# lauraset/Super-resolution-building-height-estimation

Hardware: AMD Instinct MI355X
Metric: tiles/sec (64x64x8ch->256x256 height) (higher is better)
Workload: dtype f16 operands / f32 accumulate (MFMA), f32 residual stream; 1 GPU; RRDBNet x4 (23 RRDB, 64 feat) forward_feature, batch 32 tiles/GPU, 64x64x3 -> 64x256x256 (BASELINE.json configs[1]); global_batch=32, parallelism=tile-sharded x1 (no data-path collective)

## Files before the change

super-resolution-building-height-estimation_amd/csrc/srbh_ptrunk.hip:

```cpp
#include <stdlib.h>
#include <string.h>
#include <mutex>
#include "srbh_conv3x3_kernel.h"


namespace {
using namespace srbh;
using namespace srbh_k;

struct PLayer {
    const char* w;
    const float* bias;
};

struct PParams {
    char* dense[2];
    long img_b;
    int plane_b, row_b;
    float* xr;
    float* xrr;
    const PLayer* layers;
    int nlayers;
    int H, W, tiles_per_img, nblocks;
    int* prog;
// ... 11 lines not shown
constexpr unsigned SPIN_LIMIT = 4u << 20;
using G = TileGeo<0>;
constexpr int IN_EX = G::UNITS * 16;
constexpr int A_STAGE_B = IN_EX + 18 * 1024, B_STAGE_B = IN_EX + 36 * 1024;
constexpr int A_BASE = IN_EX;
constexpr int A_BIAS_OFF = A_BASE + 2 * A_STAGE_B, B_BIAS_OFF = 2 * B_STAGE_B;
constexpr int P_WORD_OFF = A_BIAS_OFF + 128;
constexpr int P_LDS_B = 163840;
static_assert(P_WORD_OFF + 4 <= P_LDS_B && B_BIAS_OFF + 256 <= P_WORD_OFF, "LDS map must fit 160 KiB");
__device__ __forceinline__ int stage_off(int cb, int idx) { return cb == 1 ? A_BASE + idx * A_STAGE_B : idx * B_STAGE_B; }

#include "srbh_ptrunk3_kernel.h"

}

namespace srbh {

unsigned long long* g_ptrunk_prof = nullptr;
static int g_trunk_timing = 0;
static hipEvent_t g_trunk_ev[2];
static int g_trunk_ev_recorded = 0;
static const char* g_trunk_kernel = "none";

constexpr int MAX_BLOCKS = 64;
static size_t table_bytes() { return ((size_t)MAX_BLOCKS * 15 * sizeof(PLayer) + 255) & ~(size_t)255; }
static size_t prog_bytes(int B, int tpi) { return ((size_t)B * 2 * tpi * sizeof(int) + 255) & ~(size_t)255; }

size_t ptrunk_aux_bytes(int B, int tiles_per_img) { return table_bytes() + 2 * prog_bytes(B, tiles_per_img) + 256; }
__global__ void ptrunk_reset_kernel(int* __restrict__ prog, int* __restrict__ xcc, int* __restrict__ err, int n) {
    const int i = blockIdx.x * blockDim.x + threadIdx.x;
    if (i < n) { prog[i] = 0; xcc[i] = 0; }
    if (i == 0) *err = 0;
}

size_t ptrunk_err_offset(int B, int tiles_per_img) { return table_bytes() + prog_bytes(B, tiles_per_img); }

struct TabEntry {
    int dev;
    std::vector<char> host;
    PLayer* dptr;
};
static std::mutex g_tab_mu;
static std::vector<TabEntry> g_tabs;

static int device_table(const std::vector<PLayer>& tab, PLayer** out) {
    int dev = 0;
    SRBH_HIP(hipGetDevice(&dev));
    const size_t nb = tab.size() * sizeof(PLayer);
    std::lock_guard<std::mutex> lock(g_tab_mu);
    for (size_t i = 0; i < g_tabs.size(); ++i)
        if (g_tabs[i].dev == dev && g_tabs[i].host.size() == nb && memcmp(g_tabs[i].host.data(), tab.data(), nb) == 0) {
            *out = g_tabs[i].dptr;
            return SRBH_OK;
        }
    if (g_tabs.size() >= 16) {
        SRBH_HIP(hipFree(g_tabs.front().dptr));
        g_tabs.erase(g_tabs.begin());
    }
    TabEntry e;
    e.dev = dev;
    e.host.assign((const char*)tab.data(), (const char*)tab.data() + nb);
    SRBH_HIP(hipMalloc(&e.dptr, nb));
    SRBH_HIP(hipMemcpy(e.dptr, tab.data(), nb, hipMemcpyHostToDevice));
    *out = e.dptr;
    g_tabs.push_back(std::move(e));
    return SRBH_OK;
}

int ptrunk_takes(int num_block, int H, int W, int* takes, int* ncu_out) {
    *takes = 0;
    if (W != TILE_W || (H % TILE_H) != 0 || num_block <= 0 || num_block > MAX_BLOCKS) return SRBH_OK;
    int dev = 0;
    SRBH_HIP(hipGetDevice(&dev));
    int ncu = 0;
    SRBH_HIP(hipDeviceGetAttribute(&ncu, hipDeviceAttributeMultiprocessorCount, dev));
    if (ncu_out) *ncu_out = ncu;
    if (H / TILE_H > ncu) return SRBH_OK;
    constexpr int LDS_B = P_LDS_B;
    SRBH_ONCE_PER_DEVICE({
        SRBH_HIP(hipFuncSetAttribute((const void*)ptrunk3_kernel<0>, hipFuncAttributeMaxDynamicSharedMemorySize, LDS_B));
        SRBH_HIP(hipFuncSetAttribute((const void*)ptrunk3_kernel<1>, hipFuncAttributeMaxDynamicSharedMemorySize, LDS_B));
        SRBH_HIP(hipFuncSetAttribute((const void*)ptrunk3_kernel<0, 1>, hipFuncAttributeMaxDynamicSharedMemorySize, LDS_B));
        SRBH_HIP(hipFuncSetAttribute((const void*)ptrunk3_kernel<0, 0, 1>, hipFuncAttributeMaxDynamicSharedMemorySize, LDS_B));
    });
    int per_cu = 0;
    SRBH_HIP(hipOccupancyMaxActiveBlocksPerMultiprocessor(&per_cu, ptrunk3_kernel<0>, 256, LDS_B));
    if (per_cu < 1) return SRBH_OK;
    *takes = 1;
    return SRBH_OK;
}

int ptrunk_run(const srbh_rrdbnet_desc* d, void* dense0, void* dense1, float* xr, float* xrr, int B, int H, int W,
               void* aux, hipStream_t stream, int* used, int* final_cur, long train_stride, const void* mask, long mask_stride, bool bf16) {
    *used = 0;
    if (mask && train_stride <= 0) return SRBH_OK;
    SRBH_REQUIRE(!bf16 || (train_stride == 0 && !mask), "ptrunk_run: the bf16 form is the inference forward only");
    int ncu = 0, takes = 0;
    if (int rc = ptrunk_takes(d->num_block, H, W, &takes, &ncu)) return rc;
    if (!takes) return SRBH_OK;
    const int tpi = H / TILE_H;
    constexpr int LDS_B = P_LDS_B;
    const int nl = d->num_block * 15;
    std::vector<PLayer> tab(nl);
    int cur = 0, li = 0;
    for (int blk = 0; blk < d->num_block; ++blk)
        for (int r = 0; r < 3; ++r) {
            const srbh_conv_w* cw = d->rdb + (blk * 3 + r) * 5;
            for (int k = 0; k < 5; ++k) tab[li++] = PLayer{(const char*)cw[k].w, cw[k].bias};
            cur ^= 1;
        }
    *final_cur = cur;
    char* a = (char*)aux;
    PLayer* d_tab = nullptr;
    if (int rc = device_table(tab, &d_tab)) return rc;
    int* d_prog = (int*)(a + table_bytes());
    int* d_err = (int*)(a + ptrunk_err_offset(B, tpi));
    int* d_xcc = (int*)(a + ptrunk_err_offset(B, tpi) + 256);
    hipLaunchKernelGGL(ptrunk_reset_kernel, dim3((B * tpi + 255) / 256), dim3(256), 0, stream, d_prog, d_xcc, d_err, B * tpi);
    SRBH_HIP(hipGetLastError());
    const Act16Geo g = act16_geo(B, 6, H, W);
    int imgs_per_launch = ncu / tpi;
    if (const char* ie = getenv("SRBH_PT_IMAGES")) {
        const int cap = atoi(ie);
        if (cap > 0 && cap < imgs_per_launch) {
            const int nl_ = (B + cap - 1) / cap;
            imgs_per_launch = (B + nl_ - 1) / nl_;
        }
    }
    for (int b0 = 0; b0 < B; b0 += imgs_per_launch) {
        const int nb = (B - b0) < imgs_per_launch ? (B - b0) : imgs_per_launch;
        PParams pp;
        pp.dense_stride = train_stride;
        pp.keep_all = pp.out_pixel = train_stride > 0;
        pp.mask = mask ? (const char*)mask + (long)b0 * g.img_b : nullptr;
        pp.mask_stride = mask_stride;
        pp.dense[0] = (char*)dense0 + (long)b0 * g.img_b;
        pp.dense[1] = (train_stride > 0 ? (char*)dense0 + train_stride : (char*)dense1) + (long)b0 * g.img_b;
        pp.img_b = g.img_b;
        pp.plane_b = g.plane_b;
        pp.row_b = g.row_b;
        pp.xr = xr + (long)b0 * H * W * 64;
        pp.xrr = xrr + (long)b0 * H * W * 64;
        pp.layers = d_tab;
        pp.nlayers = nl;
        pp.H = H;
        pp.W = W;
        pp.tiles_per_img = tpi;
        pp.nblocks = nb * tpi;
        pp.prog = d_prog + b0 * tpi;
        pp.err = d_err;
        pp.xcc = d_xcc + b0 * tpi;
        {
            const char* e = getenv("SRBH_PT_WT");
            pp.force_wt = (e && atoi(e) == 1) ? 1 : 0;
        }
        if (getenv("SRBH_PT_PROF") && !bf16 && !g_ptrunk_prof)
            SRBH_HIP(hipMalloc(&g_ptrunk_prof, (size_t)ncu * MAX_BLOCKS * 15 * 6 * 8));
        pp.prof = bf16 ? nullptr : g_ptrunk_prof;
        if (g_trunk_timing && b0 == 0) SRBH_HIP(hipEventRecord(g_trunk_ev[0], stream));
        g_trunk_kernel = "ptrunk3_kernel";
        if (mask)
            hipLaunchKernelGGL((ptrunk3_kernel<0, 1>), dim3(pp.nblocks), dim3(256), LDS_B, stream, pp);
        else if (bf16)
            hipLaunchKernelGGL((ptrunk3_kernel<0, 0, 1>), dim3(pp.nblocks), dim3(256), LDS_B, stream, pp);
        else if (pp.prof)
            hipLaunchKernelGGL((ptrunk3_kernel<1>), dim3(pp.nblocks), dim3(256), LDS_B, stream, pp);
        else
            hipLaunchKernelGGL((ptrunk3_kernel<0>), dim3(pp.nblocks), dim3(256), LDS_B, stream, pp);
        SRBH_HIP(hipGetLastError());
    }
    if (g_trunk_timing) { SRBH_HIP(hipEventRecord(g_trunk_ev[1], stream)); g_trunk_ev_recorded = 1; }
    if (getenv("SRBH_PT_PROF") && g_ptrunk_prof && !bf16) {
        SRBH_HIP(hipStreamSynchronize(stream));
        const int nblk = (B < imgs_per_launch ? B : imgs_per_launch) * tpi;
        std::vector<unsigned long long> h((size_t)nblk * nl * 6);
        SRBH_HIP(hipMemcpy(h.data(), g_ptrunk_prof, h.size() * 8, hipMemcpyDeviceToHost));
        double cyc = 0;
        for (int b = 0; b < nblk; ++b) cyc += (double)(h[((size_t)b * nl + nl - 1) * 6 + 2] - h[(size_t)b * nl * 6]);
        fprintf(stderr, "[srbh] ptrunk: avg %.0f shader cycles per workgroup (first layer start -> last epilogue)\n", cyc / nblk);
        double loop[5] = {0}, epi[5] = {0}, pub[5] = {0}, wait[5] = {0}, tot5[5] = {0}, dma[5] = {0}, bar[5] = {0};
        for (int b = 0; b < nblk; ++b)
            for (int L = 1; L + 1 < nl; ++L) {
                const unsigned long long* q = &h[((size_t)b * nl + L) * 6];
                const unsigned long long* qn = &h[((size_t)b * nl + L + 1) * 6];
                const int k = L % 5;
                loop[k] += (double)(q[1] - q[0]); epi[k] += (double)(q[2] - q[1]); pub[k] += (double)(q[3] >> 32);
                wait[k] += (double)(q[3] & 0xffffffffu); tot5[k] += (double)(qn[0] - q[0]);
                bar[k] += (double)q[4]; dma[k] += (double)q[5];
            }
        const double cnt = (double)nblk * (nl - 2) / 5.0;
        for (int k = 0; k < 5; ++k)
            fprintf(stderr, "[srbh]   conv%d: loop %.0f (of which: waiting for the own LDS-DMA %.0f, at the step barriers %.0f; prologue %.0f) | "
                    "epilogue %.0f | publish/seam %.0f | start-to-start %.0f\n",
                    k + 1, loop[k] / cnt, dma[k] / cnt, bar[k] / cnt, wait[k] / cnt, epi[k] / cnt, pub[k] / cnt, tot5[k] / cnt);
        double e5[2] = {0, 0}, s5[2] = {0, 0};
        long n5[2] = {0, 0};
        for (int b = 0; b < nblk; ++b)
            for (int L = 4; L + 1 < nl; L += 5) {
                const unsigned long long* q = &h[((size_t)b * nl + L) * 6];
                const int kind = ((L / 5) % 3) == 2;
                e5[kind] += (double)(q[2] - q[1]); s5[kind] += (double)(q[3] >> 32); n5[kind]++;
            }
        fprintf(stderr, "[srbh]   conv5 epilogue: %.0f plain / %.0f RRDB-closing; seam %.0f / %.0f\n", e5[0] / (n5[0] ? n5[0] : 1),
                e5[1] / (n5[1] ? n5[1] : 1), s5[0] / (n5[0] ? n5[0] : 1), s5[1] / (n5[1] ? n5[1] : 1));
    }
    *used = 1;
    return SRBH_OK;
}

}

extern "C" int srbh_trunk_timing(int on) {
    using namespace srbh;
    if (on && !g_trunk_timing) {
        SRBH_HIP(hipEventCreate(&g_trunk_ev[0]));
        SRBH_HIP(hipEventCreate(&g_trunk_ev[1]));
    } else if (!on && g_trunk_timing) {
        SRBH_HIP(hipEventDestroy(g_trunk_ev[0]));
        SRBH_HIP(hipEventDestroy(g_trunk_ev[1]));
    }
    g_trunk_timing = on ? 1 : 0;
    g_trunk_ev_recorded = 0;
    return SRBH_OK;
}

extern "C" const char* srbh_trunk_kernel_name(void) { return srbh::g_trunk_kernel; }

extern "C" int srbh_trunk_last_ms(float* ms) {
    using namespace srbh;
    SRBH_REQUIRE(ms && g_trunk_timing, "srbh_trunk_last_ms: timing is off (srbh_trunk_timing(1) first)");
    SRBH_REQUIRE(g_trunk_ev_recorded, "srbh_trunk_last_ms: no persistent trunk launch was timed (per-layer path, SRBH_PERSISTENT=0?)");
    SRBH_HIP(hipEventSynchronize(g_trunk_ev[1]));
    SRBH_HIP(hipEventElapsedTime(ms, g_trunk_ev[0], g_trunk_ev[1]));
    return SRBH_OK;
}
```

super-resolution-building-height-estimation_amd/csrc/srbh_ptrunk3_kernel.h:

```cpp
#pragma once

#ifndef P3_S1
#define P3_S1 1
#endif
#ifndef P3_X2REG
#define P3_X2REG 1
#endif
#ifndef P3_SKIPST
#define P3_SKIPST 1
#endif
#ifndef P3_LAZYDRAIN
#define P3_LAZYDRAIN 1
#endif

#ifndef P3_SEAM
#define P3_SEAM 1
#endif


#ifndef P3_PREREAD
#define P3_PREREAD 1
#endif
#ifndef P3_TRAIN
#define P3_TRAIN 1
#endif
#ifndef P3_PRE_AT
#define P3_PRE_AT 2
#endif

template <int PROF, int BW = 0, int BF = 0>
__global__ __launch_bounds__(256, 1) void ptrunk3_kernel(const PParams pp) {
    extern __shared__ __attribute__((aligned(16))) char smem[];
    const int tid = threadIdx.x;
    const int lane = tid & 63;
    const int wave = __builtin_amdgcn_readfirstlane(tid >> 6);
    const int l31 = lane & 31, hi = lane >> 5;
    const int wr = wave >> 1, wc = wave & 1;
    const int t = xcd_remap(blockIdx.x, pp.nblocks);
    const int img = t / pp.tiles_per_img;
    const int ty = t - img * pp.tiles_per_img;
    const int Y0 = ty * TILE_H;
    const int up = ty > 0 ? t - 1 : -1, dn = ty + 1 < pp.tiles_per_img ? t + 1 : -1;

    int goff[G::NJ];
#pragma unroll
    for (int j = 0; j < G::NJ; ++j) {
        const int u0 = j * 256 + tid;
        const int u = u0 < G::UNITS ? u0 : 0;
        const int trow = u / (G::COLS * 4);
        const int rem = u - trow * (G::COLS * 4);
        const int pc = rem >> 2, ps = rem & 3;
        goff[j] = trow * pp.row_b + pc * PIX_B + ((ps ^ ((pc >> 2) & 3)) << 4);
    }
    const bool tail_ok = (G::NJ - 1) * 256 + tid < G::UNITS;
    int aoff[3][2];
#pragma unroll
    for (int dx = 0; dx < 3; ++dx) {
        const int pc = wc * 32 + l31 + dx;
#pragma unroll
        for (int ks = 0; ks < 2; ++ks)
            aoff[dx][ks] = wr * 4 * G::ROW_B + pc * PIX_B + (((ks * 2 + hi) ^ ((pc >> 2) & 3)) << 4);
    }
    const int woff = lane * 16;
    const long tile_off = (long)img * pp.img_b + (long)Y0 * pp.row_b;

    auto lds_addr = [](const char* p) { return (unsigned)(unsigned long long)(__attribute__((address_space(3))) const char*)p; };
    auto uni64 = [](unsigned long long m) {
        const unsigned lo = __builtin_amdgcn_readfirstlane((unsigned)m), hi32 = __builtin_amdgcn_readfirstlane((unsigned)(m >> 32));
        return ((unsigned long long)hi32 << 32) | lo;
    };
    const unsigned long long tail_mask = uni64(__builtin_amdgcn_ballot_w64(tail_ok));
    const unsigned long long w4_mask = uni64(wave < 2 ? ~0ull : 0ull);

    auto dma = [&](auto sc1_tag, const unsigned long long base, const unsigned voff, const unsigned lds_off) {
        if constexpr (decltype(sc1_tag)::value)
            asm volatile("s_mov_b32 m0, %0\n\ts_nop 3\n\tglobal_load_lds_dwordx4 %1, %2 sc1" ::"s"(lds_off), "v"(voff), "s"(base) : "memory", "m0");
        else
            asm volatile("s_mov_b32 m0, %0\n\ts_nop 3\n\tglobal_load_lds_dwordx4 %1, %2" ::"s"(lds_off), "v"(voff), "s"(base) : "memory", "m0");
    };
    auto dma_masked = [&](auto sc1_tag, const unsigned long long base, const unsigned voff, const unsigned lds_off, const unsigned long long mask) {
        if constexpr (decltype(sc1_tag)::value)
            asm volatile("s_mov_b32 m0, %1\n\ts_mov_b64 exec, %0\n\ts_nop 2\n\tglobal_load_lds_dwordx4 %2, %3 sc1\n\ts_mov_b64 exec, -1"
                         ::"s"(mask), "s"(lds_off), "v"(voff), "s"(base) : "memory", "m0");
        else
            asm volatile("s_mov_b32 m0, %1\n\ts_mov_b64 exec, %0\n\ts_nop 2\n\tglobal_load_lds_dwordx4 %2, %3\n\ts_mov_b64 exec, -1"
                         ::"s"(mask), "s"(lds_off), "v"(voff), "s"(base) : "memory", "m0");
    };
    using SC1 = std::true_type;
    using NOSC = std::false_type;
    constexpr int JORD[11] = {2, 3, 4, 5, 6, 7, 8, 0, 1, 9, 10};
    static_assert(G::NJ == 11, "DMA order is written for 11 input instructions");
    auto dma_item = [&](auto nin_tag, auto nw_tag, const int d, const unsigned long long ibase, const unsigned long long wbase,
                        const unsigned din_w, const unsigned dw_w) {
        constexpr int NIN = decltype(nin_tag)::value, NW = decltype(nw_tag)::value;
        if (d < NIN) {
            const int j = JORD[d];
            if (j < G::NJ - 1)
                dma(SC1{}, ibase, goff[j], din_w + j * 4096);
            else
                dma_masked(SC1{}, ibase, goff[j], din_w + j * 4096, uni64(tail_mask));
        } else {
            const int k = d - NIN;
            if (NW == 5 && k == 4)
                dma_masked(NOSC{}, wbase + k * 4096, woff, dw_w + k * 4096, uni64(w4_mask));
            else
                dma(NOSC{}, wbase + k * 4096, woff, dw_w + k * 4096);
        }
    };
    auto stage_cold = [&](const char* src, char* din, const char* wsrc, char* dw, auto nw_tag) {
        const unsigned long long ib = uni64((unsigned long long)src), wb = uni64((unsigned long long)(wsrc + wave * 1024));
// ... 46 lines not shown
        auto* word = (__attribute__((address_space(3))) int*)(smem);
        if (tid == 0) {
            __hip_atomic_store(pp.xcc + t, my_xcc + 1, __ATOMIC_RELAXED, __HIP_MEMORY_SCOPE_AGENT);
            int diff = pp.force_wt;
            for (int s = 0; s < 2 && !diff; ++s) {
                const int nb = s ? dn : up;
                if (nb < 0) continue;
                int v = 0;
                for (unsigned spins = 0; spins < SPIN_LIMIT; ++spins) {
                    v = __hip_atomic_load(pp.xcc + nb, __ATOMIC_RELAXED, __HIP_MEMORY_SCOPE_AGENT);
                    if (v) break;
                    __builtin_amdgcn_s_sleep(2);
                }
                if (v != my_xcc + 1) diff = 1;
            }
            *word = diff;
        }
        __syncthreads();
        wt = __builtin_amdgcn_readfirstlane(*word) != 0;
        __syncthreads();
    }
    auto publish = [&](int v) {
        if (tid == 0) {
            if (wt)
                __hip_atomic_store(pp.prog + t, v, __ATOMIC_RELAXED, __HIP_MEMORY_SCOPE_AGENT);
            else
                __hip_atomic_store(pp.prog + t, v, __ATOMIC_RELAXED, __HIP_MEMORY_SCOPE_WORKGROUP);
        }
    };
    bool pending_pub = false;
    int pub_val = 0;

    floatx4 xres[2][4][4];
    const int X = wc * 32 + l31;
    {
#pragma unroll
        for (int i = 0; i < 4; ++i) {
            const int Y = Y0 + wr * 4 + i;
            const float* q = pp.xrr + (((long)img * pp.H + Y) * pp.W + X) * 64 + hi * 4;
#pragma unroll
            for (int mb = 0; mb < 2; ++mb)
#pragma unroll
                for (int g = 0; g < 4; ++g) xres[mb][i][g] = *(const floatx4*)(q + mb * 32 + g * 8);
        }
    }

    typedef unsigned uintx4 __attribute__((ext_vector_type(4)));
    uintx4 x1p[4][2], X1r[4][2], X2r[4][2];
    const int soff = (wr * 4 + 1) * G::ROW_B + (X + 1) * PIX_B;
    const int sswz[2] = {((0 + hi) ^ (((X + 1) >> 2) & 3)) << 4, ((2 + hi) ^ (((X + 1) >> 2) & 3)) << 4};
    const int boff = (wr * 5 + (lane >> 2)) * G::ROW_B + (wc ? (G::COLS - 1) * PIX_B : 0) + (lane & 3) * 16;
    int hoff[2];
    {
        const int px = 1 + (tid >> 2), ps = tid & 3;
#pragma unroll
        for (int hrow = 0; hrow < 2; ++hrow)
            hoff[hrow] = (hrow ? G::ROWS - 1 : 0) * pp.row_b + px * PIX_B + ((ps ^ ((px >> 2) & 3)) << 4);
    }
#pragma unroll
    for (int i = 0; i < 4; ++i)
#pragma unroll
        for (int m = 0; m < 2; ++m)
            x1p[i][m] = *(const uintx4*)(pp.dense[0] + tile_off + (long)pp.plane_b + (long)(wr * 4 + i + 1) * pp.row_b + (X + 1) * PIX_B + m * 32 + hi * 16);

    auto publish_pending = [&]() {
        if (pending_pub) {
            publish(pub_val);
            pending_pub = false;
        }
    };
    unsigned long long t_sync = 0, t_vm = 0;
    auto step_sync = [&]() {
        unsigned long long w0 = 0, w1 = 0;
        if (PROF) w0 = __builtin_amdgcn_s_memtime();
        asm volatile("s_waitcnt vmcnt(0)" ::: "memory");
        if (PROF) w1 = __builtin_amdgcn_s_memtime();
        __syncthreads();
        if (PROF) {
            t_vm += w1 - w0;
            t_sync += __builtin_amdgcn_s_memtime() - w1;
        }
    };

    half8 Pq[2][G::NP], Aq[2][3][2];
    auto run_step = [&](auto cb_tag, auto in_tag, auto nw_tag, floatx16 (&acc)[decltype(cb_tag)::value][4], const char* sbi, const char* sbw,
                        const char* nsrc, const char* nw, char* dst, const uintx4 (&rsrc)[4][2], auto flag_tag, const int need,
                        auto pre_tag, auto nxt_tag) {
        constexpr int CB = decltype(cb_tag)::value, IN = decltype(in_tag)::value, NW = decltype(nw_tag)::value;
        constexpr bool FL = decltype(flag_tag)::value != 0;
        static_assert(!FL || IN != 0, "a flagged step stages an input plane");
        constexpr int NRD = G::NP + 3 * CB, NMF = 12 * CB;
        constexpr int NH = 2;
        constexpr int NDMA = (IN == 1 ? 11 : IN == 2 ? NH : 0) + NW;
        constexpr int ND = NDMA + (IN == 2 ? 9 : 0);
        static_assert(ND <= 6 * 12, "the staging items of a step must fit its MFMA shadows");
        constexpr int ORD1[9] = {6, 0, 1, 2, 3, 7, 4, 8, 5};
        constexpr int ORD2[12] = {6, 0, 7, 1, 2, 3, 8, 9, 4, 10, 11, 5};
        static_assert(G::NP == 6, "read order tables are written for 6 pixel-row fragments");
        constexpr int RSTRIDE = NMF / NRD;
        const unsigned long long ibase = uni64((unsigned long long)nsrc);
        const unsigned long long wbase = uni64((unsigned long long)(nw + wave * 1024));
        const unsigned din_w = __builtin_amdgcn_readfirstlane(lds_addr(dst) + wave * 1024);
        const unsigned dw_w = din_w + IN_EX;
        constexpr bool PRE = decltype(pre_tag)::value != 0;
        constexpr bool NXT = decltype(nxt_tag)::value != 0;
        constexpr int AT = P3_PRE_AT < NMF - NRD ? P3_PRE_AT : NMF - NRD;
        static_assert(AT >= 0, "the next step's first reads must fit behind the barrier");
        half8 (&P)[2][G::NP] = Pq;
        half8 (&A)[2][3][2] = Aq;
        auto read_from = [&](const char* bi, const char* bw, const int g, const int r, const int set) {
            const int ks = g / 3, dx = g - ks * 3;
            if (r < G::NP) {
                P[set][r] = *(const half8*)(bi + aoff[dx][ks] + r * G::ROW_B);
            } else {
                const int q = r - G::NP, dy = q / CB, mb = q - dy * CB;
                A[set][dy][mb] = *(const half8*)(bw + woff + ((((dy * 3 + dx) * 2 + ks) * CB + mb) << 10));
            }
        };
        auto read_item = [&](const int g, const int r, const int set) { read_from(sbi, sbw, g, r, set); };
        auto stage_item = [&](const int d) {
            if constexpr (FL && IN == 2) {
                if (d < NW - 1) {
                    dma_item(std::integral_constant<int, 0>{}, nw_tag, d, ibase, wbase, din_w, dw_w);
                } else if (d < NW + 7) {
                    const int e = d - (NW - 1), i = e >> 1, m = e & 1;
                    *(uintx4*)(dst + soff + sswz[m] + i * G::ROW_B) = rsrc[i][m];
                } else if (d == NW + 7) {
                    if (lane < 20) *(uintx4*)(dst + boff) = uintx4{0u, 0u, 0u, 0u};
                } else if (d == NW + 8) {
                    if (need >= 0) poll_check(std::integral_constant<int, NW - 1>{}, need);
                    dma_item(std::integral_constant<int, 0>{}, nw_tag, NW - 1, ibase, wbase, din_w, dw_w);
                } else {
                    const int h = d - NW - 9;
                    dma(SC1{}, ibase, hoff[h], din_w + (h ? G::ROWS - 1 : 0) * G::ROW_B + PIX_B);
                }
                return;
            }
            if constexpr (FL && IN == 1) {
                if (d < NW - 1) {
                    dma_item(std::integral_constant<int, 11>{}, nw_tag, d + 11, ibase, wbase, din_w, dw_w);
                } else if (d < NW + 6) {
                    dma_item(std::integral_constant<int, 11>{}, nw_tag, d - (NW - 1), ibase, wbase, din_w, dw_w);
                } else if (d == NW + 6) {
                    if (need >= 0) poll_check(std::integral_constant<int, NW + 6>{}, need);
                    dma_item(std::integral_constant<int, 11>{}, nw_tag, NW - 1 + 11, ibase, wbase, din_w, dw_w);
                } else {
                    dma_item(std::integral_constant<int, 11>{}, nw_tag, d - NW, ibase, wbase, din_w, dw_w);
                }
                return;
            }
            if constexpr (IN == 2) {
                if (d < NH) {
                    dma(SC1{}, ibase, hoff[d], din_w + (d ? G::ROWS - 1 : 0) * G::ROW_B + PIX_B);
                } else if (d < NH + NW) {
                    dma_item(std::integral_constant<int, 0>{}, nw_tag, d - NH, ibase, wbase, din_w, dw_w);
                } else if (d < NH + NW + 8) {
                    const int e = d - NH - NW, i = e >> 1, m = e & 1;
                    *(uintx4*)(dst + soff + sswz[m] + i * G::ROW_B) = rsrc[i][m];
                } else {
                    if (lane < 20) *(uintx4*)(dst + boff) = uintx4{0u, 0u, 0u, 0u};
                }
            } else {
                dma_item(std::integral_constant<int, IN == 1 ? 11 : 0>{}, nw_tag, d, ibase, wbase, din_w, dw_w);
            }
        };
        if constexpr (FL) {
            if (need >= 0) poll_issue();
        }
        if constexpr (!PRE) {
#pragma unroll
            for (int r = 0; r < NRD; ++r) read_item(0, CB == 1 ? ORD1[r % 9] : ORD2[r % 12], 0);
        }
        __builtin_amdgcn_sched_barrier(0);
#pragma unroll
        for (int g = 0; g < 6; ++g) {
#pragma unroll
            for (int m = 0; m < NMF; ++m) {
                const int dy = m / (4 * CB), rem = m - dy * 4 * CB, i = rem / CB, mb = rem - i * CB;
                if constexpr (NXT) {
                    if (g == 5 && m == AT) {
                        step_sync();
                        publish_pending();
                        __builtin_amdgcn_sched_barrier(0);
                    }
                }
                if constexpr (BW || BF)
                    acc[mb][i] = __builtin_amdgcn_mfma_f32_32x32x16_bf16(__builtin_bit_cast(bf16x8, A[g & 1][dy][mb]), __builtin_bit_cast(bf16x8, P[g & 1][i + dy]), acc[mb][i], 0, 0, 0);
                else
                    acc[mb][i] = __builtin_amdgcn_mfma_f32_32x32x16_f16(A[g & 1][dy][mb], P[g & 1][i + dy], acc[mb][i], 0, 0, 0);
                __builtin_amdgcn_sched_barrier(0);
                const int k = m / RSTRIDE;
                if (g + 1 < 6 && m % RSTRIDE == 0 && k < NRD) read_item(g + 1, CB == 1 ? ORD1[k % 9] : ORD2[k % 12], (g + 1) & 1);
                if constexpr (NXT) {
                    const int k2 = m - AT;
                    if (g == 5 && k2 >= 0 && k2 < NRD) read_from(dst, dst + IN_EX, 0, CB == 1 ? ORD1[k2 % 9] : ORD2[k2 % 12], 0);
                }
                const int sm = CB == 1 ? m : (m % 2 ? m / 2 : -1);
                if (sm >= 0) {
                    const int d = g * 12 + sm;
                    if (d < ND) stage_item(d);
                }
                __builtin_amdgcn_sched_barrier(0);
            }
        }
    };

    using C1 = std::integral_constant<int, 1>;
    using C2 = std::integral_constant<int, 2>;
    using I0 = std::integral_constant<int, 0>;
    using I1 = std::integral_constant<int, 1>;
    using I2 = std::integral_constant<int, P3_S1 ? 2 : 1>;
    using I2X = std::integral_constant<int, (P3_S1 && P3_X2REG) ? 2 : 1>;
    using W0 = std::integral_constant<int, 0>;
    using W5 = std::integral_constant<int, 5>;
    using W9 = std::integral_constant<int, 9>;
    using F0 = std::integral_constant<int, 0>;
    using F1 = std::integral_constant<int, 1>;
    using Q0 = std::integral_constant<int, 0>;
    using Q1 = std::integral_constant<int, 1>;

    auto bias_request = [&](const float* bias, const int nb) {
        float v;
        const float* q = bias + (tid < nb ? tid : 0);
        asm volatile("global_load_dword %0, %1, off" : "=v"(v) : "v"(q) : "memory");
        return v;
    };
    auto prologue_cold = [&](const float* bias, const int nb, const int bias_lds) {
        float bias_v = 0.f;
        if (tid < nb) bias_v = bias[tid];
        asm volatile("s_waitcnt vmcnt(0)" ::: "memory");
        __syncthreads();
        if (tid < nb) ((float*)(smem + bias_lds))[tid] = bias_v;
        if (pending_pub) {
            publish(pub_val);
            pending_pub = false;
        }
    };
    auto prologue = [&](auto nst_tag, const float bias_v, const int nb, const int bias_lds) {
        constexpr int NST = decltype(nst_tag)::value;
        if constexpr (NST == 8) asm volatile("s_waitcnt vmcnt(8)" ::: "memory");
        else if constexpr (NST == 2) asm volatile("s_waitcnt vmcnt(2)" ::: "memory");
        else asm volatile("s_waitcnt vmcnt(0)" ::: "memory");
        __syncthreads();
        if (tid < nb) ((float*)(smem + bias_lds))[tid] = bias_v;
    };
    auto epi32 = [&](floatx16 (&acc)[1][4], char* oplane, uintx4 (&keep)[4][2], const bool halo_only, const char* mplane = nullptr) {
        uintx4 mk[4][2];
        if constexpr (BW) {
#pragma unroll
            for (int io = 0; io < 4; ++io) {
                const int i = io == 0 ? 0 : io == 1 ? 3 : io - 1;
#pragma unroll
                for (int m = 0; m < 2; ++m)
                    mk[i][m] = *(const uintx4*)(mplane + (long)(Y0 + wr * 4 + i + 1) * pp.row_b + (X + 1) * PIX_B + m * 32 + hi * 16);
            }
        }
        floatx4 bias4[4];
#pragma unroll
        for (int g = 0; g < 4; ++g) bias4[g] = *(const floatx4*)((const float*)(smem + A_BIAS_OFF) + g * 8 + hi * 4);
#pragma unroll
        for (int io = 0; io < 4; ++io) {
            const int i = io == 0 ? 0 : io == 1 ? 3 : io - 1;
            const int Y = Y0 + wr * 4 + i;
            const bool st = !halo_only || (i == 0 && wr == 0) || (i == 3 && wr == 1);
            unsigned hp[4][2];
            if constexpr (BW) {
                unsigned mq[4][2];
#pragma unroll
                for (int m = 0; m < 2; ++m) {
                    auto u0 = __builtin_amdgcn_permlane32_swap(mk[i][m][0], mk[i][m][2], false, false);
                    auto u1 = __builtin_amdgcn_permlane32_swap(mk[i][m][1], mk[i][m][3], false, false);
                    mq[2 * m][0] = u0[0];
                    mq[2 * m + 1][0] = u0[1];
                    mq[2 * m][1] = u1[0];
                    mq[2 * m + 1][1] = u1[1];
                }
#pragma unroll
                for (int g = 0; g < 4; ++g) {
                    const half4 mh = __builtin_bit_cast(half4, uint2{mq[g][0], mq[g][1]});
                    unsigned r[4];
#pragma unroll
                    for (int q = 0; q < 4; ++q) {
                        float w = acc[0][i][g * 4 + q];
                        w = (float)mh[q] > 0.f ? w : w * 0.2f;
                        const unsigned u = __builtin_bit_cast(unsigned, w);
                        r[q] = (u + 0x7fffu + ((u >> 16) & 1u)) >> 16;
                    }
                    hp[g][0] = r[0] | (r[1] << 16);
                    hp[g][1] = r[2] | (r[3] << 16);
                }
            } else {
#pragma unroll
            for (int g = 0; g < 4; ++g) {
                floatx4 w;
#pragma unroll
                for (int q = 0; q < 4; ++q) w[q] = acc[0][i][g * 4 + q];
                w += bias4[g];
                const floatx4 ws = w * 0.2f;
#pragma unroll
                for (int q = 0; q < 4; ++q) asm("v_max_f32 %0, %1, %2" : "=v"(w[q]) : "v"(w[q]), "v"(ws[q]));
                if constexpr (BF) {
                    hp[g][0] = bf16x2_rne(w[0], w[1]);
                    hp[g][1] = bf16x2_rne(w[2], w[3]);
                } else {
                half4 h4;
#pragma unroll
                for (int q = 0; q < 4; ++q) h4[q] = (_Float16)w[q];
                const uint2 u = __builtin_bit_cast(uint2, h4);
                hp[g][0] = u.x;
                hp[g][1] = u.y;
                }
            }
            }
#pragma unroll
            for (int m = 0; m < 2; ++m) {
                auto s0 = __builtin_amdgcn_permlane32_swap(hp[2 * m][0], hp[2 * m + 1][0], false, false);
                auto s1 = __builtin_amdgcn_permlane32_swap(hp[2 * m][1], hp[2 * m + 1][1], false, false);
                const uintx4 raw = {s0[0], s1[0], s0[1], s1[1]};
                keep[i][m] = raw;
                char* o = oplane + (long)(Y + 1) * pp.row_b + (X + 1) * PIX_B + m * 32 + hi * 16;
                if (st) {
                    if (wt)
                        asm volatile("global_store_dwordx4 %0, %1, off sc1\n\ts_nop 1" ::"v"(o), "v"(raw) : "memory");
                    else
                        asm volatile("global_store_dwordx4 %0, %1, off\n\ts_nop 1" ::"v"(o), "v"(raw) : "memory");
                }
            }
        }
    };
    auto x_row_out = [&](const int mb, const int i, char* obase, const bool st, const bool to_lds, const bool f16out) {
        const int Y = Y0 + wr * 4 + i;
        unsigned hp[4][2];
#pragma unroll
        for (int g = 0; g < 4; ++g) {
            if constexpr (BW) {
                unsigned r[4];
#pragma unroll
                for (int q = 0; q < 4; ++q) {
                    const float xv = xres[mb][i][g][q];
                    const unsigned u = __builtin_bit_cast(unsigned, xv);
                    r[q] = (u + 0x7fffu + ((u >> 16) & 1u)) >> 16;
                }
                hp[g][0] = r[0] | (r[1] << 16);
                hp[g][1] = r[2] | (r[3] << 16);
            } else if (BF && !f16out) {
                hp[g][0] = bf16x2_rne(xres[mb][i][g][0], xres[mb][i][g][1]);
                hp[g][1] = bf16x2_rne(xres[mb][i][g][2], xres[mb][i][g][3]);
            } else {
                half4 h4;
#pragma unroll
                for (int q = 0; q < 4; ++q) h4[q] = (_Float16)xres[mb][i][g][q];
                const uint2 u = __builtin_bit_cast(uint2, h4);
                hp[g][0] = u.x;
                hp[g][1] = u.y;
            }
        }
#pragma unroll
        for (int m = 0; m < 2; ++m) {
            auto s0 = __builtin_amdgcn_permlane32_swap(hp[2 * m][0], hp[2 * m + 1][0], false, false);
            auto s1 = __builtin_amdgcn_permlane32_swap(hp[2 * m][1], hp[2 * m + 1][1], false, false);
            const uintx4 raw = {s0[0], s1[0], s0[1], s1[1]};
            if (mb == 1) x1p[i][m] = raw;
            if (P3_SEAM && mb == 0 && to_lds) *(uintx4*)(smem + soff + sswz[m] + i * G::ROW_B) = raw;
            char* o = obase + (long)mb * pp.plane_b + (long)(Y + 1) * pp.row_b + (X + 1) * PIX_B + m * 32 + hi * 16;
            if (st) {
                if (wt)
                    asm volatile("global_store_dwordx4 %0, %1, off sc1\n\ts_nop 1" ::"v"(o), "v"(raw) : "memory");
                else
                    asm volatile("global_store_dwordx4 %0, %1, off\n\ts_nop 1" ::"v"(o), "v"(raw) : "memory");
            }
        }
    };
    auto epi64 = [&](floatx16 (&acc)[2][4], char* obase, const bool r2, const bool r2_pixel, const bool x1_halo_only, const bool keep, const bool out_px,
                     const bool f16out) {
        floatx4 bias4[2][4];
#pragma unroll
        for (int mb = 0; mb < 2; ++mb)
#pragma unroll
            for (int g = 0; g < 4; ++g) bias4[mb][g] = *(const floatx4*)((const float*)(smem + B_BIAS_OFF) + mb * 32 + g * 8 + hi * 4);
        const int frag_lane = wc * 2048 + lane * 4;
        floatx4 a2[2][2][4];
        auto load_a2 = [&](const int slot, const int i) {
            const long rowb = ((long)img * pp.H + Y0 + wr * 4 + i) * pp.W * 64;
            const float* q2 = pp.xrr + rowb + (r2_pixel ? X * 64 + hi * 4 : frag_lane);
            const int sm = r2_pixel ? 32 : 1024, sg = r2_pixel ? 8 : 256;
#pragma unroll
            for (int mb = 0; mb < 2; ++mb)
#pragma unroll
                for (int g = 0; g < 4; ++g) a2[slot][mb][g] = *(const floatx4*)(q2 + mb * sm + g * sg);
        };
#pragma unroll
        for (int io = 0; io < 4; ++io) {
            const int i = io == 0 ? 0 : io == 1 ? 3 : io - 1;
            if (r2 && io == 1) load_a2(0, 0);
            if (r2 && io == 2) load_a2(1, 3);
            const bool halo = (i == 0 && wr == 0) || (i == 3 && wr == 1);
#pragma unroll
            for (int mb = 0; mb < 2; ++mb) {
#pragma unroll
                for (int g = 0; g < 4; ++g) {
                    floatx4 tt;
#pragma unroll
                    for (int q = 0; q < 4; ++q) tt[q] = acc[mb][i][g * 4 + q];
                    tt += bias4[mb][g];
                    xres[mb][i][g] = tt * 0.2f + xres[mb][i][g];
                }
                if (!r2) x_row_out(mb, i, obase, keep || (!P3_SEAM && mb == 0) || !x1_halo_only || halo, x1_halo_only, f16out);
            }
        }
        if (r2) {
            auto close_row = [&](const int slot, const int i) {
                const bool halo = (i == 0 && wr == 0) || (i == 3 && wr == 1);
                const long rowb = ((long)img * pp.H + Y0 + wr * 4 + i) * pp.W * 64;
#pragma unroll
                for (int mb = 0; mb < 2; ++mb) {
#pragma unroll
                    for (int g = 0; g < 4; ++g) xres[mb][i][g] = xres[mb][i][g] * 0.2f + a2[slot][mb][g];
                    x_row_out(mb, i, obase, keep || (!P3_SEAM && mb == 0) || !x1_halo_only || halo, x1_halo_only, f16out);
                }
                const float* q = (out_px ? pp.xr : pp.xrr) + rowb;
                const unsigned vo = out_px ? (unsigned)(X * 64 + hi * 4) * 4u : (unsigned)frag_lane * 4u;
#pragma unroll
                for (int mb = 0; mb < 2; ++mb)
#pragma unroll
                    for (int g = 0; g < 4; ++g) {
                        const unsigned long long sb = uni64((unsigned long long)(q + (out_px ? mb * 32 + g * 8 : mb * 1024 + g * 256)));
                        asm volatile("s_nop 4\n\tglobal_store_dwordx4 %0, %1, %2\n\ts_nop 1" ::"v"(vo), "v"(xres[mb][i][g]), "s"(sb) : "memory");
                    }
            };
            close_row(0, 0);
            load_a2(0, 1);
            close_row(1, 3);
            load_a2(1, 2);
            close_row(0, 1);
            close_row(1, 2);
        }
    };

    char* dcur = pp.dense[0] + tile_off;
    char* dnxt = pp.dense[1] + tile_off;
    const char* mcur = BW ? pp.mask + tile_off : nullptr;
    stage_cold(dcur, smem, pp.layers[0].w, smem + stage_off(1, 0) + (P3_SEAM ? 0 : IN_EX), W5{});
    const int nrdb = pp.nlayers / 5;
    for (int rdb = 0; rdb < nrdb; ++rdb) {
        const PLayer* T = pp.layers + rdb * 5;
        const int L0 = rdb * 5;
        int gs = 0;
        float next_bias = 0.f;
        auto layerA = [&](auto kk_tag, auto last_nw_tag) {
            constexpr int kk = decltype(kk_tag)::value;
            const int L = L0 + kk, n = kk + 2;
            const char* wl = T[kk].w;
            unsigned long long p0 = 0, p1 = 0, p2 = 0;
            if (PROF) p0 = __builtin_amdgcn_s_memtime();
            if (P3_LAZYDRAIN && kk > 0) {
                constexpr bool prev_halo_only = P3_SKIPST && P3_S1 && (kk - 1 == 0 || (P3_X2REG && kk - 1 == 1));
                prologue(std::integral_constant<int, prev_halo_only ? 2 : 8>{}, next_bias, 32, A_BIAS_OFF);
            } else {
                prologue_cold(T[kk].bias, 32, A_BIAS_OFF);
            }
            if (PROF) p1 = __builtin_amdgcn_s_memtime();
            t_sync = 0;
            t_vm = 0;
            floatx16 acc[1][4];
#pragma unroll
            for (int i = 0; i < 4; ++i)
#pragma unroll
                for (int r = 0; r < 16; ++r) acc[0][i][r] = 0.f;
            run_step(C1{}, I2{}, W5{}, acc, smem, smem + stage_off(1, gs & 1) + ((P3_SEAM && kk == 0) ? 0 : IN_EX), dcur + (long)pp.plane_b, wl + 18 * 1024,
                     smem + stage_off(1, (gs + 1) & 1), x1p, F0{}, 0, Q0{}, Q1{});
            ++gs;
            if (n >= 3) {
                const char* st = smem + stage_off(1, gs & 1);
                run_step(C1{}, I2{}, W5{}, acc, st, st + IN_EX, dcur + 2l * pp.plane_b, wl + 2 * (18 * 1024),
                         smem + stage_off(1, (gs + 1) & 1), X1r, std::integral_constant<int, kk == 1>{}, L, Q1{}, Q1{});
                ++gs;
            }
            if (n >= 4) {
                const char* st = smem + stage_off(1, gs & 1);
                run_step(C1{}, I2X{}, W5{}, acc, st, st + IN_EX, dcur + 3l * pp.plane_b, wl + 3 * (18 * 1024),
                         smem + stage_off(1, (gs + 1) & 1), X2r, std::integral_constant<int, kk == 2>{}, L, Q1{}, Q1{});
                ++gs;
            }
            if (n >= 5) {
                const char* st = smem + stage_off(1, gs & 1);
                run_step(C1{}, I1{}, W5{}, acc, st, st + IN_EX, dcur + 4l * pp.plane_b, wl + 4 * (18 * 1024),
                         smem + stage_off(1, (gs + 1) & 1), x1p, F1{}, L, Q1{}, Q1{});
                ++gs;
            }
            {
                const char* st = smem + stage_off(1, gs & 1);
                if constexpr (decltype(last_nw_tag)::value == 5)
                    run_step(C1{}, I0{}, W5{}, acc, st, st + IN_EX, nullptr, T[kk + 1].w, smem + stage_off(1, (gs + 1) & 1), x1p, F0{}, 0, Q1{}, Q0{});
                else
                    run_step(C1{}, I0{}, W9{}, acc, st, st + IN_EX, nullptr, T[4].w, smem + stage_off(2, 0), x1p, F0{}, 0, Q1{}, Q0{});
                ++gs;
            }
            if (P3_LAZYDRAIN) next_bias = bias_request(T[kk + 1].bias, kk == 3 ? 64 : 32);
            if (PROF) p2 = __builtin_amdgcn_s_memtime();
            uintx4 kept[4][2];
            const bool halo_only = P3_SKIPST && P3_S1 && (kk == 0 || (P3_X2REG && kk == 1)) && !(P3_TRAIN && pp.keep_all);
            epi32(acc, dcur + (long)(2 + kk) * pp.plane_b - (long)Y0 * pp.row_b, kept, halo_only,
                  BW ? mcur + (long)(5 - kk) * pp.plane_b - (long)Y0 * pp.row_b : nullptr);
            if (kk == 0) {
#pragma unroll
                for (int io = 0; io < 4; ++io)
#pragma unroll
                    for (int m = 0; m < 2; ++m) X1r[io][m] = kept[io][m];
            }
            if (kk == 1) {
#pragma unroll
                for (int io = 0; io < 4; ++io)
#pragma unroll
                    for (int m = 0; m < 2; ++m) X2r[io][m] = kept[io][m];
            }
            pending_pub = true;
            pub_val = L + 1;
            if (PROF && tid == 0) {
                unsigned long long* q = pp.prof + ((long)blockIdx.x * pp.nlayers + L) * 6;
                q[0] = p1; q[1] = p2; q[2] = __builtin_amdgcn_s_memtime(); q[3] = p1 - p0; q[4] = t_sync; q[5] = t_vm;
            }
        };
        layerA(std::integral_constant<int, 0>{}, W5{});
        layerA(std::integral_constant<int, 1>{}, W5{});
        layerA(std::integral_constant<int, 2>{}, W5{});
        layerA(std::integral_constant<int, 3>{}, W9{});
        {
            const int L = L0 + 4;
            const char* wl = T[4].w;
            unsigned long long p0 = 0, p1 = 0, p2 = 0, p3 = 0;
            if (PROF) p0 = __builtin_amdgcn_s_memtime();
            if (P3_LAZYDRAIN) {
                prologue(std::integral_constant<int, 8>{}, next_bias, 64, B_BIAS_OFF);
            } else {
                prologue_cold(T[4].bias, 64, B_BIAS_OFF);
            }
            if (PROF) p1 = __builtin_amdgcn_s_memtime();
            t_sync = 0;
            t_vm = 0;
            floatx16 acc[2][4];
#pragma unroll
            for (int mb = 0; mb < 2; ++mb)
#pragma unroll
                for (int i = 0; i < 4; ++i)
#pragma unroll
                    for (int r = 0; r < 16; ++r) acc[mb][i][r] = 0.f;
            {
                const char* st = smem + stage_off(2, 0);
                run_step(C2{}, I2{}, W9{}, acc, st, st + IN_EX, dcur + (long)pp.plane_b, wl + 36 * 1024, smem + stage_off(2, 1), x1p, F0{}, 0, Q0{}, Q1{});
            }
            {
                const char* st = smem + stage_off(2, 1);
                run_step(C2{}, I2{}, W9{}, acc, st, st + IN_EX, dcur + 2l * pp.plane_b, wl + 2 * (36 * 1024), smem + stage_off(2, 0), X1r, F0{}, 0, Q1{}, Q1{});
            }
            {
                const char* st = smem + stage_off(2, 0);
                run_step(C2{}, I2X{}, W9{}, acc, st, st + IN_EX, dcur + 3l * pp.plane_b, wl + 3 * (36 * 1024), smem + stage_off(2, 1), X2r, F0{}, 0, Q1{}, Q1{});
            }
            {
                int c = 3;
                do {
                    const char* st = smem + stage_off(2, c & 1);
                    run_step(C2{}, I1{}, W9{}, acc, st, st + IN_EX, dcur + (long)(c + 1) * pp.plane_b, wl + (long)(c + 1) * (36 * 1024),
                             smem + stage_off(2, (c + 1) & 1), x1p, F1{}, c == 4 ? L : -1, Q1{}, Q1{});
                } while (++c < 5);
            }
            {
                const char* st = smem + stage_off(2, 1);
                if constexpr (P3_SEAM) {
                    const char* nw5 = rdb + 1 < nrdb ? T[5].w : T[0].w;
                    run_step(C2{}, I0{}, W5{}, acc, st, st + IN_EX, nullptr, nw5, smem, x1p, F0{}, 0, Q1{}, Q0{});
                } else {
                    run_step(C2{}, I0{}, W0{}, acc, st, st + IN_EX, nullptr, nullptr, smem, x1p, F0{}, 0, Q1{}, Q0{});
                }
            }
            const bool r2 = (rdb % 3) == 2;
            if (PROF) p2 = __builtin_amdgcn_s_memtime();
            epi64(acc, dnxt - (long)Y0 * pp.row_b, r2, rdb == 2, P3_SKIPST && P3_S1 && rdb + 1 < nrdb, P3_TRAIN && pp.keep_all != 0,
                  P3_TRAIN && pp.out_pixel != 0 && rdb + 1 == nrdb, BF && rdb + 1 == nrdb);
            if (PROF) p3 = __builtin_amdgcn_s_memtime();
            asm volatile("s_waitcnt vmcnt(0)" ::: "memory");
            __syncthreads();
            publish(L + 1);
            if (rdb + 1 < nrdb) {
                poll_issue();
                poll_check(std::integral_constant<int, 0>{}, L + 1);
                if constexpr (P3_SEAM) {
                    const unsigned long long ib = uni64((unsigned long long)dnxt);
                    const unsigned din_w = __builtin_amdgcn_readfirstlane(lds_addr(smem) + wave * 1024);
                    dma(SC1{}, ib, hoff[0], din_w + PIX_B);
                    dma(SC1{}, ib, hoff[1], din_w + (G::ROWS - 1) * G::ROW_B + PIX_B);
                } else {
                    stage_cold(dnxt, smem, T[5].w, smem + stage_off(1, 0) + IN_EX, W5{});
                }
            }
            if (PROF && tid == 0) {
                unsigned long long* q = pp.prof + ((long)blockIdx.x * pp.nlayers + L) * 6;
                q[0] = p1; q[1] = p2; q[2] = p3; q[3] = (p1 - p0) | ((unsigned long long)(__builtin_amdgcn_s_memtime() - p3) << 32); q[4] = t_sync; q[5] = t_vm;
            }
            if constexpr (BW) mcur += pp.mask_stride;
            if (P3_TRAIN && pp.dense_stride) {
                dcur = dnxt;
                dnxt = dnxt + pp.dense_stride;
            } else {
                char* tmp = dcur;
                dcur = dnxt;
                dnxt = tmp;
            }
        }
    }
}
```

Baseline: 8201 tiles/s.

## Defer RRDB-closing xrr residual stores into next RDB's conv1-2 K loops

Instead of storing the f32 RRDB residual stream (xrr) to global memory in the conv5 epilogue of an RRDB-closing RDB, the epilogue now returns early. The stores are issued later as masked global_store_dwordx4 instructions interleaved at fixed slots inside the cout-32 conv1/conv2 K-loop steps of the following RDB, so they overlap with MFMA work rather than lengthening the epilogue. It relies on the step barrier's vmcnt(0) to cover them. It also extends profiling to the bf16 path and adds per-RDB cycle breakdown output. The cost is more accumulator-register pressure to keep xres alive across steps and more complex scheduling constraints.

```diff
diff --git a/super-resolution-building-height-estimation_amd/csrc/srbh_ptrunk.hip b/super-resolution-building-height-estimation_amd/csrc/srbh_ptrunk.hip
--- a/super-resolution-building-height-estimation_amd/csrc/srbh_ptrunk.hip
+++ b/super-resolution-building-height-estimation_amd/csrc/srbh_ptrunk.hip
@@ -117,6 +117,7 @@
         SRBH_HIP(hipFuncSetAttribute((const void*)ptrunk3_kernel<1>, hipFuncAttributeMaxDynamicSharedMemorySize, LDS_B));
         SRBH_HIP(hipFuncSetAttribute((const void*)ptrunk3_kernel<0, 1>, hipFuncAttributeMaxDynamicSharedMemorySize, LDS_B));
         SRBH_HIP(hipFuncSetAttribute((const void*)ptrunk3_kernel<0, 0, 1>, hipFuncAttributeMaxDynamicSharedMemorySize, LDS_B));
+        SRBH_HIP(hipFuncSetAttribute((const void*)ptrunk3_kernel<1, 0, 1>, hipFuncAttributeMaxDynamicSharedMemorySize, LDS_B));
     });
     int per_cu = 0;
     SRBH_HIP(hipOccupancyMaxActiveBlocksPerMultiprocessor(&per_cu, ptrunk3_kernel<0>, 256, LDS_B));
@@ -189,13 +190,15 @@
             const char* e = getenv("SRBH_PT_WT");
             pp.force_wt = (e && atoi(e) == 1) ? 1 : 0;
         }
-        if (getenv("SRBH_PT_PROF") && !bf16 && !g_ptrunk_prof)
+        if (getenv("SRBH_PT_PROF") && !mask && !g_ptrunk_prof)
             SRBH_HIP(hipMalloc(&g_ptrunk_prof, (size_t)ncu * MAX_BLOCKS * 15 * 6 * 8));
-        pp.prof = bf16 ? nullptr : g_ptrunk_prof;
+        pp.prof = mask ? nullptr : g_ptrunk_prof;
         if (g_trunk_timing && b0 == 0) SRBH_HIP(hipEventRecord(g_trunk_ev[0], stream));
         g_trunk_kernel = "ptrunk3_kernel";
         if (mask)
             hipLaunchKernelGGL((ptrunk3_kernel<0, 1>), dim3(pp.nblocks), dim3(256), LDS_B, stream, pp);
+        else if (bf16 && pp.prof)
+            hipLaunchKernelGGL((ptrunk3_kernel<1, 0, 1>), dim3(pp.nblocks), dim3(256), LDS_B, stream, pp);
         else if (bf16)
             hipLaunchKernelGGL((ptrunk3_kernel<0, 0, 1>), dim3(pp.nblocks), dim3(256), LDS_B, stream, pp);
         else if (pp.prof)
@@ -205,7 +208,7 @@
         SRBH_HIP(hipGetLastError());
     }
     if (g_trunk_timing) { SRBH_HIP(hipEventRecord(g_trunk_ev[1], stream)); g_trunk_ev_recorded = 1; }
-    if (getenv("SRBH_PT_PROF") && g_ptrunk_prof && !bf16) {
+    if (getenv("SRBH_PT_PROF") && g_ptrunk_prof && !mask) {
         SRBH_HIP(hipStreamSynchronize(stream));
         const int nblk = (B < imgs_per_launch ? B : imgs_per_launch) * tpi;
         std::vector<unsigned long long> h((size_t)nblk * nl * 6);
@@ -238,6 +241,17 @@
             }
         fprintf(stderr, "[srbh]   conv5 epilogue: %.0f plain / %.0f RRDB-closing; seam %.0f / %.0f\n", e5[0] / (n5[0] ? n5[0] : 1),
                 e5[1] / (n5[1] ? n5[1] : 1), s5[0] / (n5[0] ? n5[0] : 1), s5[1] / (n5[1] ? n5[1] : 1));
+        double rd[3] = {0, 0, 0}, l13[3] = {0, 0, 0};
+        long nr[3] = {0, 0, 0};
+        for (int b = 0; b < nblk; ++b)
+            for (int r = 1; r + 1 < nl / 5; ++r) {
+                const unsigned long long* q = &h[((size_t)b * nl + r * 5) * 6];
+                rd[r % 3] += (double)(q[5 * 6] - q[0]); nr[r % 3]++;
+                for (int k = 0; k < 3; ++k) l13[r % 3] += (double)(q[k * 6 + 1] - q[k * 6]);
+            }
+        for (int k = 0; k < 3; ++k)
+            fprintf(stderr, "[srbh]   RDB %d of an RRDB: %.0f cycles, of which the K loops of conv1..conv3 %.0f\n", k + 1, rd[k] / (nr[k] ? nr[k] : 1),
+                    l13[k] / (nr[k] ? nr[k] : 1));
     }
     *used = 1;
     return SRBH_OK;
diff --git a/super-resolution-building-height-estimation_amd/csrc/srbh_ptrunk3_kernel.h b/super-resolution-building-height-estimation_amd/csrc/srbh_ptrunk3_kernel.h
--- a/super-resolution-building-height-estimation_amd/csrc/srbh_ptrunk3_kernel.h
+++ b/super-resolution-building-height-estimation_amd/csrc/srbh_ptrunk3_kernel.h
@@ -26,6 +26,9 @@
 #endif
 #ifndef P3_PRE_AT
 #define P3_PRE_AT 2
+#endif
+#ifndef P3_XRRLATE
+#define P3_XRRLATE 1
 #endif
 
 template <int PROF, int BW = 0, int BF = 0>
@@ -238,11 +241,29 @@
         }
     };
 
+    constexpr bool XL = P3_XRRLATE && !BW;
+    static_assert(!XL || TILE_W == 64, "fragment order of the stream: two waves of 32 pixels per row");
+    unsigned long long xl_base = 0;
+    if constexpr (XL) xl_base = uni64((unsigned long long)(pp.xrr + ((long)img * pp.H + Y0 + wr * 4) * TILE_W * 64 + wc * 2048));
+    unsigned long long xl_mask = 0;
+    auto xl_store = [&](const unsigned long long m, const unsigned long long sb, const int i, const int e) {
+        const int mb = e >> 2, g = e & 3;
+#define P3_XL_ST(OFF) asm volatile("s_mov_b64 exec, %0\n\tglobal_store_dwordx4 %1, %2, %3 offset:" #OFF "\n\ts_mov_b64 exec, -1" \
+                                   ::"s"(m), "v"(woff), "a"(xres[mb][i][g]), "s"(sb) : "memory")
+        if (g == 0) P3_XL_ST(0);
+        else if (g == 1) P3_XL_ST(1024);
+        else if (g == 2) P3_XL_ST(2048);
+        else P3_XL_ST(3072);
+#undef P3_XL_ST
+    };
+
     half8 Pq[2][G::NP], Aq[2][3][2];
     auto run_step = [&](auto cb_tag, auto in_tag, auto nw_tag, floatx16 (&acc)[decltype(cb_tag)::value][4], const char* sbi, const char* sbw,
                         const char* nsrc, const char* nw, char* dst, const uintx4 (&rsrc)[4][2], auto flag_tag, const int need,
-                        auto pre_tag, auto nxt_tag) {
+                        auto pre_tag, auto nxt_tag, auto xq_tag) {
         constexpr int CB = decltype(cb_tag)::value, IN = decltype(in_tag)::value, NW = decltype(nw_tag)::value;
+        constexpr int XQ = XL ? decltype(xq_tag)::value : -1;
+        constexpr int XD[8] = {21, 22, 23, 33, 34, 35, 45, 46};
         constexpr bool FL = decltype(flag_tag)::value != 0;
         static_assert(!FL || IN != 0, "a flagged step stages an input plane");
         constexpr int NRD = G::NP + 3 * CB, NMF = 12 * CB;
@@ -262,6 +283,8 @@
         constexpr bool NXT = decltype(nxt_tag)::value != 0;
         constexpr int AT = P3_PRE_AT < NMF - NRD ? P3_PRE_AT : NMF - NRD;
         static_assert(AT >= 0, "the next step's first reads must fit behind the barrier");
+        static_assert(XQ < 0 || (CB == 1 && NXT && !FL && ND <= XD[0] && XD[7] < 5 * 12 + AT),
+                      "deferred stores: a cout-32 step without a neighbour check, all of them in front of its barrier (whose vmcnt(0) covers them)");
         half8 (&P)[2][G::NP] = Pq;
         half8 (&A)[2][3][2] = Aq;
         auto read_from = [&](const char* bi, const char* bw, const int g, const int r, const int set) {
@@ -320,6 +343,12 @@
                 dma_item(std::integral_constant<int, IN == 1 ? 11 : 0>{}, nw_tag, d, ibase, wbase, din_w, dw_w);
             }
         };
+        unsigned long long xl_m = 0, xl_b0 = 0, xl_b1 = 0;
+        if constexpr (XQ >= 0) {
+            xl_m = uni64(xl_mask);
+            xl_b0 = uni64(xl_base) + (unsigned)(XQ * TILE_W * 64 * 4);
+            xl_b1 = xl_b0 + 4096;
+        }
         if constexpr (FL) {
             if (need >= 0) poll_issue();
         }
@@ -355,6 +384,11 @@
                 if (sm >= 0) {
                     const int d = g * 12 + sm;
                     if (d < ND) stage_item(d);
+                    if constexpr (XQ >= 0) {
+#pragma unroll
+                        for (int e = 0; e < 8; ++e)
+                            if (d == XD[e]) xl_store(xl_m, e < 4 ? xl_b0 : xl_b1, XQ, e);
+                    }
                 }
                 __builtin_amdgcn_sched_barrier(0);
             }
@@ -374,6 +408,7 @@
     using F1 = std::integral_constant<int, 1>;
     using Q0 = std::integral_constant<int, 0>;
     using Q1 = std::integral_constant<int, 1>;
+    using XN = std::integral_constant<int, -1>;
 
     auto bias_request = [&](const float* bias, const int nb) {
         float v;
@@ -528,7 +563,7 @@
         }
     };
     auto epi64 = [&](floatx16 (&acc)[2][4], char* obase, const bool r2, const bool r2_pixel, const bool x1_halo_only, const bool keep, const bool out_px,
-                     const bool f16out) {
+                     const bool f16out, const bool xrr_late) {
         floatx4 bias4[2][4];
 #pragma unroll
         for (int mb = 0; mb < 2; ++mb)
@@ -574,6 +609,7 @@
                     for (int g = 0; g < 4; ++g) xres[mb][i][g] = xres[mb][i][g] * 0.2f + a2[slot][mb][g];
                     x_row_out(mb, i, obase, keep || (!P3_SEAM && mb == 0) || !x1_halo_only || halo, x1_halo_only, f16out);
                 }
+                if (XL && xrr_late) return;
                 const float* q = (out_px ? pp.xr : pp.xrr) + rowb;
                 const unsigned vo = out_px ? (unsigned)(X * 64 + hi * 4) * 4u : (unsigned)frag_lane * 4u;
 #pragma unroll
@@ -624,32 +660,33 @@
 #pragma unroll
                 for (int r = 0; r < 16; ++r) acc[0][i][r] = 0.f;
             run_step(C1{}, I2{}, W5{}, acc, smem, smem + stage_off(1, gs & 1) + ((P3_SEAM && kk == 0) ? 0 : IN_EX), dcur + (long)pp.plane_b, wl + 18 * 1024,
-                     smem + stage_off(1, (gs + 1) & 1), x1p, F0{}, 0, Q0{}, Q1{});
+                     smem + stage_off(1, (gs + 1) & 1), x1p, F0{}, 0, Q0{}, Q1{}, std::integral_constant<int, kk <= 2 ? kk : -1>{});
             ++gs;
             if (n >= 3) {
                 const char* st = smem + stage_off(1, gs & 1);
                 run_step(C1{}, I2{}, W5{}, acc, st, st + IN_EX, dcur + 2l * pp.plane_b, wl + 2 * (18 * 1024),
-                         smem + stage_off(1, (gs + 1) & 1), X1r, std::integral_constant<int, kk == 1>{}, L, Q1{}, Q1{});
+                         smem + stage_off(1, (gs + 1) & 1), X1r, std::integral_constant<int, kk == 1>{}, L, Q1{}, Q1{},
+                         std::integral_constant<int, kk == 2 ? 3 : -1>{});
                 ++gs;
             }
             if (n >= 4) {
                 const char* st = smem + stage_off(1, gs & 1);
                 run_step(C1{}, I2X{}, W5{}, acc, st, st + IN_EX, dcur + 3l * pp.plane_b, wl + 3 * (18 * 1024),
-                         smem + stage_off(1, (gs + 1) & 1), X2r, std::integral_constant<int, kk == 2>{}, L, Q1{}, Q1{});
+                         smem + stage_off(1, (gs + 1) & 1), X2r, std::integral_constant<int, kk == 2>{}, L, Q1{}, Q1{}, XN{});
                 ++gs;
             }
             if (n >= 5) {
                 const char* st = smem + stage_off(1, gs & 1);
                 run_step(C1{}, I1{}, W5{}, acc, st, st + IN_EX, dcur + 4l * pp.plane_b, wl + 4 * (18 * 1024),
-                         smem + stage_off(1, (gs + 1) & 1), x1p, F1{}, L, Q1{}, Q1{});
+                         smem + stage_off(1, (gs + 1) & 1), x1p, F1{}, L, Q1{}, Q1{}, XN{});
                 ++gs;
             }
             {
                 const char* st = smem + stage_off(1, gs & 1);
                 if constexpr (decltype(last_nw_tag)::value == 5)
-                    run_step(C1{}, I0{}, W5{}, acc, st, st + IN_EX, nullptr, T[kk + 1].w, smem + stage_off(1, (gs + 1) & 1), x1p, F0{}, 0, Q1{}, Q0{});
+                    run_step(C1{}, I0{}, W5{}, acc, st, st + IN_EX, nullptr, T[kk + 1].w, smem + stage_off(1, (gs + 1) & 1), x1p, F0{}, 0, Q1{}, Q0{}, XN{});
                 else
-                    run_step(C1{}, I0{}, W9{}, acc, st, st + IN_EX, nullptr, T[4].w, smem + stage_off(2, 0), x1p, F0{}, 0, Q1{}, Q0{});
+                    run_step(C1{}, I0{}, W9{}, acc, st, st + IN_EX, nullptr, T[4].w, smem + stage_off(2, 0), x1p, F0{}, 0, Q1{}, Q0{}, XN{});
                 ++gs;
             }
             if (P3_LAZYDRAIN) next_bias = bias_request(T[kk + 1].bias, kk == 3 ? 64 : 32);
@@ -703,37 +740,38 @@
                     for (int r = 0; r < 16; ++r) acc[mb][i][r] = 0.f;
             {
                 const char* st = smem + stage_off(2, 0);
-                run_step(C2{}, I2{}, W9{}, acc, st, st + IN_EX, dcur + (long)pp.plane_b, wl + 36 * 1024, smem + stage_off(2, 1), x1p, F0{}, 0, Q0{}, Q1{});
+                run_step(C2{}, I2{}, W9{}, acc, st, st + IN_EX, dcur + (long)pp.plane_b, wl + 36 * 1024, smem + stage_off(2, 1), x1p, F0{}, 0, Q0{}, Q1{}, XN{});
             }
             {
                 const char* st = smem + stage_off(2, 1);
-                run_step(C2{}, I2{}, W9{}, acc, st, st + IN_EX, dcur + 2l * pp.plane_b, wl + 2 * (36 * 1024), smem + stage_off(2, 0), X1r, F0{}, 0, Q1{}, Q1{});
+                run_step(C2{}, I2{}, W9{}, acc, st, st + IN_EX, dcur + 2l * pp.plane_b, wl + 2 * (36 * 1024), smem + stage_off(2, 0), X1r, F0{}, 0, Q1{}, Q1{}, XN{});
             }
             {
                 const char* st = smem + stage_off(2, 0);
-                run_step(C2{}, I2X{}, W9{}, acc, st, st + IN_EX, dcur + 3l * pp.plane_b, wl + 3 * (36 * 1024), smem + stage_off(2, 1), X2r, F0{}, 0, Q1{}, Q1{});
+                run_step(C2{}, I2X{}, W9{}, acc, st, st + IN_EX, dcur + 3l * pp.plane_b, wl + 3 * (36 * 1024), smem + stage_off(2, 1), X2r, F0{}, 0, Q1{}, Q1{}, XN{});
             }
             {
                 int c = 3;
                 do {
                     const char* st = smem + stage_off(2, c & 1);
                     run_step(C2{}, I1{}, W9{}, acc, st, st + IN_EX, dcur + (long)(c + 1) * pp.plane_b, wl + (long)(c + 1) * (36 * 1024),
-                             smem + stage_off(2, (c + 1) & 1), x1p, F1{}, c == 4 ? L : -1, Q1{}, Q1{});
+                             smem + stage_off(2, (c + 1) & 1), x1p, F1{}, c == 4 ? L : -1, Q1{}, Q1{}, XN{});
                 } while (++c < 5);
             }
             {
                 const char* st = smem + stage_off(2, 1);
                 if constexpr (P3_SEAM) {
                     const char* nw5 = rdb + 1 < nrdb ? T[5].w : T[0].w;
-                    run_step(C2{}, I0{}, W5{}, acc, st, st + IN_EX, nullptr, nw5, smem, x1p, F0{}, 0, Q1{}, Q0{});
+                    run_step(C2{}, I0{}, W5{}, acc, st, st + IN_EX, nullptr, nw5, smem, x1p, F0{}, 0, Q1{}, Q0{}, XN{});
                 } else {
-                    run_step(C2{}, I0{}, W0{}, acc, st, st + IN_EX, nullptr, nullptr, smem, x1p, F0{}, 0, Q1{}, Q0{});
+                    run_step(C2{}, I0{}, W0{}, acc, st, st + IN_EX, nullptr, nullptr, smem, x1p, F0{}, 0, Q1{}, Q0{}, XN{});
                 }
             }
             const bool r2 = (rdb % 3) == 2;
             if (PROF) p2 = __builtin_amdgcn_s_memtime();
             epi64(acc, dnxt - (long)Y0 * pp.row_b, r2, rdb == 2, P3_SKIPST && P3_S1 && rdb + 1 < nrdb, P3_TRAIN && pp.keep_all != 0,
-                  P3_TRAIN && pp.out_pixel != 0 && rdb + 1 == nrdb, BF && rdb + 1 == nrdb);
+                  P3_TRAIN && pp.out_pixel != 0 && rdb + 1 == nrdb, BF && rdb + 1 == nrdb, rdb + 1 < nrdb);
+            if constexpr (XL) xl_mask = (r2 && rdb + 1 < nrdb) ? ~0ull : 0ull;
             if (PROF) p3 = __builtin_amdgcn_s_memtime();
             asm volatile("s_waitcnt vmcnt(0)" ::: "memory");
             __syncthreads();
```

Measured after the change: 8157 tiles/s, median of 2. No clear change (-0.5%).
